# fverdoja/Fast-3D-Pointcloud-Segmentation

Measured on AMD Instinct MI355X. Metric: Mpoints/sec segmented end-to-end, 1M-pt RGB-D frames, higher is better.
Workload: dtype f32

## Files before the change

fast-3d-pointcloud-segmentation_amd/csrc/f3ds_kernels.inc:

```


namespace {

struct P16 { float x, y, z; uint32_t rgba; };

struct DevCounters {
    unsigned long long n_finite;
    uint32_t bbox[6];
    uint32_t bbox_any;
    uint32_t n_valid;
    uint32_t n_voxels;
    uint32_t n_cells;
    uint32_t n_seeds;
    uint32_t n_edges;
    uint32_t n_alive;
    uint32_t n_merges;
    uint32_t n_regions;
    uint32_t n_events;
    int error;
    int r_overflow;
    float lambda;
    uint32_t seg_count;
    uint32_t n_ghosts;
    int depth;
// ... 94 lines not shown
            uint32_t v[16];
            if (i0 + 15u < m) {
#pragma unroll
                for (int q = 0; q < 4; ++q) { const uint4 x = *reinterpret_cast<const uint4*>(data + i0 + 4 * q); v[4 * q] = x.x; v[4 * q + 1] = x.y; v[4 * q + 2] = x.z; v[4 * q + 3] = x.w; }
            } else {
#pragma unroll
                for (int k = 0; k < 16; ++k) v[k] = i0 + k < m ? data[i0 + k] : 0u;
            }
            uint32_t sum = 0;
#pragma unroll
            for (int k = 0; k < 16; ++k) sum += v[k];
            uint32_t tot;
            const uint32_t inc = block_incl_scan<256>(sum, &tot);
            uint32_t run = carry + inc - sum;
            if (i0 + 15u < m) {
#pragma unroll
                for (int q = 0; q < 4; ++q) {
                    uint4 x; x.x = run; x.y = run + v[4 * q]; x.z = x.y + v[4 * q + 1]; x.w = x.z + v[4 * q + 2]; run = x.w + v[4 * q + 3];
                    *reinterpret_cast<uint4*>(data + i0 + 4 * q) = x;
                }
            } else {
#pragma unroll
                for (int k = 0; k < 16; ++k) if (i0 + k < m) { data[i0 + k] = run; run += v[k]; }
            }
            carry += tot;
        }
    }
};
struct d_scan_tiles {
    static constexpr int BLOCK = SCAN_THREADS;
    __device__ void operator()(const uint32_t* in, uint32_t* out, uint32_t* tile_sums, uint32_t n) const {
        if (BIX > 0 && BIX * SCAN_TILE >= n) return;
        const uint32_t base = BIX * SCAN_TILE + threadIdx.x * SCAN_ITEMS;
        uint32_t v[SCAN_ITEMS];
        uint32_t s = 0;
    #pragma unroll
        for (int i = 0; i < SCAN_ITEMS; ++i) { v[i] = (base + i < n) ? in[base + i] : 0u; s += v[i]; }
        uint32_t tot;
        uint32_t inc = block_incl_scan<SCAN_THREADS>(s, &tot);
        uint32_t run = inc - s;
    #pragma unroll
        for (int i = 0; i < SCAN_ITEMS; ++i) { run += v[i]; if (base + i < n) out[base + i] = run; }
        if (threadIdx.x == 0) tile_sums[BIX] = tot;
    }
};
struct d_scan_add {
    static constexpr int BLOCK = SCAN_THREADS;
    __device__ void operator()(uint32_t* out, const uint32_t* tile_offsets, uint32_t n) const {
        if (BIX > 0 && BIX * SCAN_TILE >= n) return;
        const uint32_t base = BIX * SCAN_TILE + threadIdx.x * SCAN_ITEMS;
        const uint32_t off = tile_offsets[BIX];
    #pragma unroll
        for (int i = 0; i < SCAN_ITEMS; ++i) if (base + i < n) out[base + i] += off;
    }
};

constexpr int RS_THREADS = 256;
constexpr int RS_WAVES = RS_THREADS / 64;
constexpr int RS_STRIPS = 16;
constexpr int RS_TILE = RS_THREADS * RS_STRIPS;
constexpr int RS_MAXBITS = 9;
constexpr int RS_BINS = 1 << RS_MAXBITS;

struct d_radix_hist {
    static constexpr int BLOCK = RS_THREADS;
    __device__ void operator()(const uint64_t* keys, uint32_t n, int shift, int bits, uint32_t* hist,
                                                         uint32_t nblocks, const uint32_t* n_dev) const {
        if (BIX >= nblocks) return;
        if (n_dev) { const uint32_t nd = *n_dev; n = nd < n ? nd : n; }
        __shared__ uint32_t lh[RS_BINS];
        for (int i = threadIdx.x; i < RS_BINS; i += RS_THREADS) lh[i] = 0;
        __syncthreads();
        const uint32_t mask = (1u << bits) - 1u;
        const uint32_t wbase = BIX * RS_TILE + (threadIdx.x >> 6) * (64 * RS_STRIPS);
    #pragma unroll
        for (int s = 0; s < RS_STRIPS; ++s) {
            uint32_t i = wbase + s * 64 + lane_id();
            if (i < n) atomicAdd(&lh[(uint32_t)(keys[i] >> shift) & mask], 1u);
        }
        __syncthreads();
        for (uint32_t d = threadIdx.x; d < (1u << bits); d += RS_THREADS) hist[d * nblocks + BIX] = lh[d];
    }
};
struct d_radix_scatter {
    static constexpr int BLOCK = RS_THREADS;
    __device__ void operator()(const uint64_t* keys, const uint32_t* vals, uint64_t* keys_out,
                                                            uint32_t* vals_out, uint32_t n, int shift, int bits,
                                                            const uint32_t* hist_scanned, uint32_t nblocks, const uint32_t* n_dev) const {
        if (BIX >= nblocks) return;
        if (n_dev) { const uint32_t nd = *n_dev; n = nd < n ? nd : n; }
        __shared__ uint32_t wcount[RS_WAVES][RS_BINS];
        const uint32_t mask = (1u << bits) - 1u;
        const int w = threadIdx.x >> 6;
        for (int i = threadIdx.x; i < RS_WAVES * RS_BINS; i += RS_THREADS) (&wcount[0][0])[i] = 0;
        __syncthreads();
        const uint32_t wbase = BIX * RS_TILE + w * (64 * RS_STRIPS);
        uint64_t k[RS_STRIPS];
    #pragma unroll
        for (int s = 0; s < RS_STRIPS; ++s) {
            uint32_t i = wbase + s * 64 + lane_id();
            k[s] = i < n ? keys[i] : 0ull;
            if (i < n) atomicAdd(&wcount[w][(uint32_t)(k[s] >> shift) & mask], 1u);
        }
        __syncthreads();
        for (uint32_t d = threadIdx.x; d < (1u << bits); d += RS_THREADS) {
            uint32_t run = hist_scanned[d * nblocks + BIX];
            for (int ww = 0; ww < RS_WAVES; ++ww) { uint32_t t = wcount[ww][d]; wcount[ww][d] = run; run += t; }
        }
        __syncthreads();
    #pragma unroll
        for (int s = 0; s < RS_STRIPS; ++s) {
            uint32_t i = wbase + s * 64 + lane_id();
            const bool valid = i < n;
            const uint32_t d = (uint32_t)(k[s] >> shift) & mask;
            uint64_t peers = __ballot(valid);
            for (int b = 0; b < bits; ++b) {
                uint64_t m = __ballot(valid && ((d >> b) & 1u));
                peers &= ((d >> b) & 1u) ? m : ~m;
            }
            uint32_t pos = 0;
            if (valid) pos = wcount[w][d] + (uint32_t)__popcll(peers & lanemask_lt());
            __builtin_amdgcn_wave_barrier();
            if (valid && (peers & lanemask_lt()) == 0ull) wcount[w][d] += (uint32_t)__popcll(peers);
            __builtin_amdgcn_wave_barrier();
            if (valid) { keys_out[pos] = k[s]; vals_out[pos] = vals[i]; }
        }
    }
};


struct d_radix_scatter_k {
    static constexpr int BLOCK = RS_THREADS;
    __device__ void operator()(const uint64_t* keys, uint64_t* keys_out, uint32_t n, int shift, int bits, const uint32_t* hist_scanned, uint32_t nblocks) const {
        if (BIX >= nblocks) return;
        __shared__ uint32_t wcount[RS_WAVES][RS_BINS];
        const uint32_t mask = (1u << bits) - 1u;
        const int w = threadIdx.x >> 6;
        for (int i = threadIdx.x; i < RS_WAVES * RS_BINS; i += RS_THREADS) (&wcount[0][0])[i] = 0;
        __syncthreads();
        const uint32_t wbase = BIX * RS_TILE + w * (64 * RS_STRIPS);
        uint64_t k[RS_STRIPS];
    #pragma unroll
        for (int s = 0; s < RS_STRIPS; ++s) {
            uint32_t i = wbase + s * 64 + lane_id();
            k[s] = i < n ? keys[i] : 0ull;
            if (i < n) atomicAdd(&wcount[w][(uint32_t)(k[s] >> shift) & mask], 1u);
        }
        __syncthreads();
        for (uint32_t d = threadIdx.x; d < (1u << bits); d += RS_THREADS) {
            uint32_t run = hist_scanned[d * nblocks + BIX];
            for (int ww = 0; ww < RS_WAVES; ++ww) { uint32_t t = wcount[ww][d]; wcount[ww][d] = run; run += t; }
        }
        __syncthreads();
    #pragma unroll
        for (int s = 0; s < RS_STRIPS; ++s) {
            uint32_t i = wbase + s * 64 + lane_id();
            const bool valid = i < n;
            const uint32_t d = (uint32_t)(k[s] >> shift) & mask;
            uint64_t peers = __ballot(valid);
            for (int b = 0; b < bits; ++b) {
                uint64_t m = __ballot(valid && ((d >> b) & 1u));
                peers &= ((d >> b) & 1u) ? m : ~m;
            }
            uint32_t pos = 0;
            if (valid) pos = wcount[w][d] + (uint32_t)__popcll(peers & lanemask_lt());
            __builtin_amdgcn_wave_barrier();
            if (valid && (peers & lanemask_lt()) == 0ull) wcount[w][d] += (uint32_t)__popcll(peers);
            __builtin_amdgcn_wave_barrier();
            if (valid) keys_out[pos] = k[s];
        }
    }
};

struct FrameArgs {
    int use_transform, fold_negative_z, leaf_order;
    float voxel_res, seed_res, w_color, w_spatial, w_normal;
};

__device__ inline P16 load_point(const P16* pts, size_t i) {
    const uint4 q = reinterpret_cast<const uint4*>(pts)[i];
    P16 p;
    p.x = __uint_as_float(q.x); p.y = __uint_as_float(q.y); p.z = __uint_as_float(q.z); p.rgba = q.w;
    return p;
}

__device__ inline bool vt_blocks(int depth) { return depth <= N_BLOCK_DEPTH_MAX; }
constexpr uint32_t BT_EMPTY = 0xFFFFFFFFu;
struct __attribute__((aligned(16))) BtEntry { uint32_t key, base; unsigned long long vacant; };
static_assert(sizeof(BtEntry) == 16, "one 16-byte load per probe");
template <class T> __device__ inline bool vt_cas(T* p, T* expect, T v, bool agent) {
    return agent ? __hip_atomic_compare_exchange_strong(p, expect, v, __ATOMIC_RELAXED, __ATOMIC_RELAXED, __HIP_MEMORY_SCOPE_AGENT)
                 : __hip_atomic_compare_exchange_strong(p, expect, v, __ATOMIC_RELAXED, __ATOMIC_RELAXED, __HIP_MEMORY_SCOPE_WORKGROUP);
}
__device__ inline void vt_insert(uint64_t* hkeys, uint32_t* hvals, uint32_t hmask, bool agent, unsigned x, unsigned y, unsigned z, uint32_t v) {
    const unsigned long long pk = (unsigned long long)n_pack_key(x, y, z);
    uint32_t h = (uint32_t)hash64((uint64_t)pk) & hmask;
    for (;;) {
        unsigned long long expect = HASH_EMPTY;
        if (vt_cas((unsigned long long*)&hkeys[h], &expect, pk, agent) || expect == pk) { hvals[h] = v; return; }
        h = (h + 1u) & hmask;
    }
}
__device__ inline int vt_find(const uint64_t* hkeys, const uint32_t* hvals, uint32_t hmask, unsigned x, unsigned y, unsigned z) {
    const uint64_t pk = n_pack_key(x, y, z);
    uint32_t h = (uint32_t)hash64(pk) & hmask;
    for (;;) {
        const uint64_t k = hkeys[h];
        if (k == pk) return (int)hvals[h];
        if (k == HASH_EMPTY) return -1;
        h = (h + 1u) & hmask;
    }
}
__device__ inline BtEntry* bt_entry(BtEntry* tab, uint32_t tmask, bool agent, uint32_t bk) {
    uint32_t h = (uint32_t)hash64((uint64_t)bk) & tmask;
    for (;;) {
        uint32_t expect = BT_EMPTY;
        if (vt_cas(&tab[h].key, &expect, bk, agent) || expect == bk) return &tab[h];
        h = (h + 1u) & tmask;
    }
}
__device__ inline int bt_find(const BtEntry* tab, uint32_t tmask, int leaf_order, unsigned x, unsigned y, unsigned z) {
    const uint32_t bk = n_block_key(x, y, z);
    uint32_t h = (uint32_t)hash64((uint64_t)bk) & tmask;
    for (;;) {
        const uint4 e = reinterpret_cast<const uint4*>(tab)[h];
        if (e.x == bk) return n_block_ordinal(e.y, ~(((uint64_t)e.w << 32) | (uint64_t)e.z), n_block_cell(x, y, z), leaf_order);
        if (e.x == BT_EMPTY) return -1;
        h = (h + 1u) & tmask;
    }
}
struct RgbdArgs {
    uint32_t width, n;
    uint32_t depth_pitch, color_pitch;
    int depth_f32, color_format;
    float depth_scale, fx, fy, cx, cy;
};
template <class T> __device__ inline T load_unaligned(const unsigned char* p) { T t; __builtin_memcpy(&t, p, sizeof(T)); return t; }
template <bool DEPTH_F32, int COLOR>
__device__ inline void deproject_loop(const unsigned char* depth, const unsigned char* color, const RgbdArgs& a, P16* out) {
    const uint32_t stride = gridDim.x * blockDim.x;
    const uint32_t sv = stride / a.width, su = stride - sv * a.width;
    uint32_t i = BIX * blockDim.x + threadIdx.x;
    uint32_t v = i / a.width, u = i - v * a.width;
    for (; i < a.n; i += stride) {
        const unsigned char* drow = depth + (size_t)v * a.depth_pitch;
        const unsigned char* crow = color + (size_t)v * a.color_pitch;
        float z = 0.0f;
        bool valid;
        if constexpr (DEPTH_F32) valid = n_depth_to_z(reinterpret_cast<const float*>(drow)[u], a.depth_scale, z);
        else valid = n_depth_to_z(reinterpret_cast<const uint16_t*>(drow)[u], a.depth_scale, z);
        uint32_t rgba;
        if constexpr (COLOR == 0) { const unsigned char* p = crow + 3u * (size_t)u; rgba = n_color_word(p[0], p[1], p[2], 255u); }
        else {
            const uint32_t w = load_unaligned<uint32_t>(crow + 4u * (size_t)u);
            rgba = COLOR == 1 ? n_color_word(w & 255u, (w >> 8) & 255u, (w >> 16) & 255u, w >> 24) : w;
        }
        float x, y, zo;
        n_deproject(u, v, valid, z, a.fx, a.fy, a.cx, a.cy, x, y, zo);
        reinterpret_cast<uint4*>(out)[i] = make_uint4(__float_as_uint(x), __float_as_uint(y), __float_as_uint(zo), rgba);
        u += su; v += sv;
        if (u >= a.width) { u -= a.width; ++v; }
    }
}
struct d_deproject {
    static constexpr int BLOCK = 256;
    __device__ void operator()(const unsigned char* depth, const unsigned char* color, RgbdArgs a, P16* out) const {
        if (a.depth_f32) {
            if (a.color_format == 0) deproject_loop<true, 0>(depth, color, a, out);
            else if (a.color_format == 1) deproject_loop<true, 1>(depth, color, a, out);
            else deproject_loop<true, 2>(depth, color, a, out);
        } else {
            if (a.color_format == 0) deproject_loop<false, 0>(depth, color, a, out);
            else if (a.color_format == 1) deproject_loop<false, 1>(depth, color, a, out);
            else deproject_loop<false, 2>(depth, color, a, out);
        }
    }
};
struct d_bbox {
    static constexpr int BLOCK = 256;
    __device__ void operator()(const P16* pts, uint32_t n, FrameArgs fa, DevCounters* dc) const {
        float mn[3] = {F3DS_FLT_MAX, F3DS_FLT_MAX, F3DS_FLT_MAX}, mx[3] = {-F3DS_FLT_MAX, -F3DS_FLT_MAX, -F3DS_FLT_MAX};
        uint32_t nfin = 0, any = 0;
        for (uint32_t i = BIX * blockDim.x + threadIdx.x; i < n; i += gridDim.x * blockDim.x) {
            P16 p = load_point(pts, i);
            float x = p.x, y = p.y, z = p.z;
            n_prelude(z, fa.fold_negative_z);
            if (n_finite3(x, y, z)) nfin++;
            n_transform(x, y, z, fa.use_transform);
            if (!n_finite3(x, y, z)) continue;
            any = 1;
            if (x < mn[0]) mn[0] = x;
            if (y < mn[1]) mn[1] = y;
            if (z < mn[2]) mn[2] = z;
            if (x > mx[0]) mx[0] = x;
            if (y > mx[1]) mx[1] = y;
            if (z > mx[2]) mx[2] = z;
        }
    #pragma unroll
        for (int d = 32; d >= 1; d >>= 1) {
            for (int a = 0; a < 3; ++a) {
                float t = __shfl_xor(mn[a], d, 64); if (t < mn[a]) mn[a] = t;
                t = __shfl_xor(mx[a], d, 64); if (t > mx[a]) mx[a] = t;
            }
            nfin += __shfl_xor(nfin, d, 64);
            any |= __shfl_xor(any, d, 64);
        }
        __shared__ float smn[4][3], smx[4][3];
        __shared__ uint32_t sfin[4], sany[4];
        const int w = threadIdx.x >> 6;
        if (lane_id() == 0) { for (int a = 0; a < 3; ++a) { smn[w][a] = mn[a]; smx[w][a] = mx[a]; } sfin[w] = nfin; sany[w] = any; }
// ... 513 lines not shown
                    const unsigned long long o = __shfl_down(m, d, 64);
                    if (lane + d < 64u && !(ahead & ((1ull << d) - 1ull))) m |= o;
                }
                if (in && (head || lane == 0u)) {
                    BtEntry* const e = bt_entry(tab, hmask, agent, bk);
                    if (agent) __hip_atomic_fetch_and(&e->vacant, ~m, __ATOMIC_RELAXED, __HIP_MEMORY_SCOPE_AGENT);
                    else __hip_atomic_fetch_and(&e->vacant, ~m, __ATOMIC_RELAXED, __HIP_MEMORY_SCOPE_WORKGROUP);
                    if (head) e->base = v;
                }
            }
        }
    }
};
struct d_voxel_list_accum {
    static constexpr int BLOCK = 256;
    __device__ void operator()(const P16* pts, uint32_t* list, const uint32_t* seg_start, FrameArgs fa, float* vf, uint32_t* vcount, DevCounters* dc, uint32_t capV) const {
        __shared__ __attribute__((aligned(16))) uint4 buf[VG_CHUNK];
        if (dc->ev_overflow) return;
        const uint32_t V = dc->n_voxels < capV ? dc->n_voxels : capV;
        const bool disorder = dc->vox_disorder != 0u;
        const uint32_t tid = threadIdx.x;
        for (uint32_t vb = BIX * 256u; vb < V; vb += gridDim.x * 256u) {
            const uint32_t v = vb + tid;
            const bool mine = v < V;
            const uint32_t s = mine ? seg_start[v] : 0u, e = mine ? seg_start[v + 1] : 0u;
            const uint32_t p0 = seg_start[vb], p1 = seg_start[vb + 256u < V ? vb + 256u : V];
            if (__syncthreads_or(e - s > VL_MAX_RUN)) { if (tid == 0) { dc->error = F3DS_ERR_UNSUPPORTED; dc->ev_overflow = 6; } return; }
            if (disorder) {
                for (uint32_t a = s + 1u; a < e; ++a) {
                    const uint32_t x = list[a];
                    uint32_t b = a;
                    while (b > s && list[b - 1u] > x) { list[b] = list[b - 1u]; --b; }
                    if (b != a) list[b] = x;
                }
                __threadfence_block();
                __syncthreads();
            }
            float sx = 0, sy = 0, sz = 0, sr = 0, sg = 0, sb = 0;
            for (uint32_t c0 = p0; c0 < p1; c0 += VG_CHUNK) {
                const uint32_t c1 = p1 - c0 < VG_CHUNK ? p1 : c0 + VG_CHUNK;
                uint32_t idx[VG_CHUNK / 256];
        #pragma unroll
                for (uint32_t j = 0; j < VG_CHUNK / 256; ++j) { const uint32_t i = c0 + j * 256u + tid; idx[j] = list[i < c1 ? i : c1 - 1u]; }
                uint4 q[VG_CHUNK / 256];
        #pragma unroll
                for (uint32_t j = 0; j < VG_CHUNK / 256; ++j) q[j] = reinterpret_cast<const uint4*>(pts)[idx[j]];
        #pragma unroll
                for (uint32_t j = 0; j < VG_CHUNK / 256; ++j) buf[j * 256u + tid] = q[j];
                __syncthreads();
                const uint32_t a = s > c0 ? s : c0, b = e < c1 ? e : c1;
                for (uint32_t i = a; i < b; ++i) {
                    const uint4 w = buf[i - c0];
                    float z = __uint_as_float(w.z); n_prelude(z, fa.fold_negative_z);
                    sx += __uint_as_float(w.x); sy += __uint_as_float(w.y); sz += z;
                    sr += (float)((w.w >> 16) & 255u); sg += (float)((w.w >> 8) & 255u); sb += (float)(w.w & 255u);
                }
                __syncthreads();
            }
            if (!mine) continue;
            const float c = (float)(e - s);
            vcount[v] = e - s;
            float4* row = reinterpret_cast<float4*>(vf + (size_t)v * 12);
            row[0] = make_float4(sx / c, sy / c, sz / c, sr / c);
            row[1] = make_float4(sg / c, sb / c, 0.0f, 0.0f);
            row[2] = make_float4(0.0f, 0.0f, 0.0f, 0.0f);
        }
    }
};
__device__ inline int hash_find(const uint64_t* hkeys, const uint32_t* hvals, uint32_t hmask, uint64_t pk) {
    uint32_t h = (uint32_t)hash64(pk) & hmask;
    for (;;) {
        uint64_t k = hkeys[h];
        if (k == pk) return (int)hvals[h];
        if (k == HASH_EMPTY) return -1;
        h = (h + 1u) & hmask;
    }
}

struct d_neighbors {
    static constexpr int BLOCK = 256;
    __device__ void operator()(const uint32_t* vkey, const DevCounters* dc, const GridInfo* gp, int leaf_order, const uint64_t* hkeys,
                                                  const uint32_t* hvals, uint32_t hmask, int* nbr, int* nbrT) const {
        __shared__ int tr[27][65];
        const uint32_t V = dc->n_voxels;
        const unsigned max_key = gp->max_key;
        const bool blocks = vt_blocks(gp->depth);
        const BtEntry* const tab = reinterpret_cast<const BtEntry*>(hkeys);
        for (uint32_t vb = BIX * 64u; vb < V; vb += gridDim.x * 64u) {
            const uint32_t nv = V - vb < 64u ? V - vb : 64u, np = nv * 27u;
            for (uint32_t tl = threadIdx.x; tl < np; tl += 256u) {
                const uint32_t vl = tl / 27u, s = tl - vl * 27u, v = vb + vl;
                const int d[3] = {(int)(s / 9u) - 1, (int)((s / 3u) % 3u) - 1, (int)(s % 3u) - 1};
                bool ok = true; unsigned k[3];
                for (int a = 0; a < 3; ++a) {
                    long long q = (long long)vkey[v * 3 + a] + d[a];
                    if (q < 0 || q > (long long)max_key) ok = false;
                    k[a] = (unsigned)q;
                }
                const int u = !ok ? -1 : blocks ? bt_find(tab, hmask, leaf_order, k[0], k[1], k[2]) : vt_find(hkeys, hvals, hmask, k[0], k[1], k[2]);
                nbr[(size_t)vb * 27u + tl] = u;
                tr[s][vl] = u;
            }
            __syncthreads();
            for (uint32_t r = threadIdx.x; r < 27u * 64u; r += 256u) {
                const uint32_t s = r >> 6, vl = r & 63u;
                if (vl < nv) nbrT[(size_t)s * V + vb + vl] = tr[s][vl];
            }
            __syncthreads();
        }
    }
};
constexpr int NT_TILE = 128;
constexpr int NT_HCAP = 2048;
#ifndef F3DS_NT_SLOTS
#define F3DS_NT_SLOTS 896
#endif
#ifndef F3DS_NT_RING1
#define F3DS_NT_RING1 448
#endif
constexpr int NT_SLOTS = F3DS_NT_SLOTS;
constexpr int NT_RING1 = F3DS_NT_RING1;
constexpr uint16_t NT_NONE = 0xFFFFu;
constexpr uint32_t NT_HNONE = 0x3FFu;
constexpr uint32_t NT_ORD_LIMIT = (1u << 22) - 2u;
static_assert(NT_SLOTS < 1023, "slot numbers share a word with the ordinal");
constexpr uint16_t NT_ZERO = NT_SLOTS;
constexpr uint32_t SW_TILE_NONE = 0xFFFFFFFFu;
constexpr int SW_SLOT_BITS = 9;
constexpr int SW_SLOT_WORDS = (27 * SW_SLOT_BITS + 31) / 32;
static_assert(NT_RING1 < (1 << SW_SLOT_BITS), "a list position must fit its bit field");
__device__ __forceinline__ void sw_slots_pack(const uint32_t pos[27], uint32_t w[SW_SLOT_WORDS]) {
#pragma unroll
    for (int k = 0; k < SW_SLOT_WORDS; ++k) w[k] = 0u;
#pragma unroll
    for (int j = 0; j < 27; ++j) {
        const int bit = j * SW_SLOT_BITS, wi = bit >> 5, sh = bit & 31;
        w[wi] |= pos[j] << sh;
        if (sh + SW_SLOT_BITS > 32) w[wi + 1] |= pos[j] >> (32 - sh);
    }
}
__device__ __forceinline__ uint32_t sw_slot(const uint32_t w[SW_SLOT_WORDS], int j) {
    const int bit = j * SW_SLOT_BITS, wi = bit >> 5, sh = bit & 31;
    uint32_t x = w[wi] >> sh;
    if (sh + SW_SLOT_BITS > 32) x |= w[wi + 1] << (32 - sh);
    return x & ((1u << SW_SLOT_BITS) - 1u);
}
__device__ inline void cov_add(float acc[9], const float4 q) {
    acc[0] += q.x * q.x; acc[1] += q.x * q.y; acc[2] += q.x * q.z;
    acc[3] += q.y * q.y; acc[4] += q.y * q.z; acc[5] += q.z * q.z;
    acc[6] += q.x; acc[7] += q.y; acc[8] += q.z;
}
__device__ __forceinline__ uint32_t lds_addr(const float* p);
typedef float f3ds_f2 __attribute__((ext_vector_type(2)));
typedef float f3ds_f4 __attribute__((ext_vector_type(4)));
struct CovPairs {
    f3ds_f2 a0, a1, a2, a3; float sz;
    __device__ void zero() { a0 = a1 = a2 = a3 = f3ds_f2{0.0f, 0.0f}; sz = 0.0f; }
    __device__ void add(const f3ds_f4 q) {
        const f3ds_f2 xy = q.xy, zy = q.zw;
        a0 += xy * q.xx;
        a1 += xy * q.zz;
        a2 += zy * zy;
        a3 += xy;
        sz += q.z;
    }
    __device__ void store(float acc[9]) const { acc[0] = a0.x; acc[1] = a0.y; acc[2] = a1.x; acc[3] = a2.y; acc[4] = a1.y; acc[5] = a2.x; acc[6] = a3.x; acc[7] = a3.y; acc[8] = sz; }
};
template <int NTT>
struct d_normals_t {
    static constexpr int BLOCK = NTT;
    static constexpr int PT = (NT_RING1 * 27 + NTT - 1) / NTT;
    static constexpr int PR = PT % 9 == 0 ? 9 : (PT % 8 == 0 ? 8 : (PT % 6 == 0 ? 6 : (PT % 4 == 0 ? 4 : (PT % 3 == 0 ? 3 : (PT % 2 == 0 ? 2 : 1)))));
#ifndef F3DS_NORMALS_WPS
#define F3DS_NORMALS_WPS 3
#endif
#ifndef F3DS_NORMALS_WPS256
#define F3DS_NORMALS_WPS256 3
#endif
    static constexpr int WAVES_PER_SIMD = NTT > 256 ? F3DS_NORMALS_WPS : F3DS_NORMALS_WPS256;
    __device__ static uint32_t hslot(uint32_t ord) { return (ord * 2654435761u) >> 21; }
    __device__ void one_tile(const uint32_t bix, float* vf, const int* nbr, const DevCounters* dc, uint32_t* tile_n1, uint32_t* tile_ord, uint32_t* tile_slots, uint32_t holes) const {
        __shared__ uint32_t hw[NT_HCAP];
// ... 2987 lines not shown
```

fast-3d-pointcloud-segmentation_amd/csrc/f3ds_numerics.h:

```cpp
#ifndef F3DS_NUMERICS_H_
#define F3DS_NUMERICS_H_

#include "f3ds_math.h"

namespace f3ds {

#define F3DS_FLT_MAX 3.402823466e+38f
#define F3DS_FLT_MIN 1.175494351e-38f
#define F3DS_FLT_EPS 1.192092896e-07f

F3DS_HD float n_sqrtf(float x) { return __builtin_sqrtf(x); }
F3DS_HD double n_sqrt(double x) { return __builtin_sqrt(x); }
F3DS_HD bool n_finite3(float x, float y, float z) { return m_isfinitef(x) && m_isfinitef(y) && m_isfinitef(z); }
F3DS_HD float n_nanf() { return m_from_bitsf(0x7fc00000u); }

struct GridInfo {
    double min[3];
    double max[3];
    double res;
    int depth;
    unsigned max_key;
    int error;
    int empty;
};
// ... 31 lines not shown
        if (k > mk) mk = k;
    }
    double lg = m_log((double)mk) / m_log(2.0) - eps;
    unsigned d = (unsigned)__builtin_ceil(lg);
    if (d > 32u) d = 32u;
    if (d > 21u) { g.error = -4; g.depth = (int)d; return; }
    g.depth = (int)d;
    g.max_key = (1u << d) - 1u;
    double side = (double)(1u << d) * g.res;
    for (int a = 0; a < 3; ++a) {
        double over = (side - (g.max[a] - g.min[a])) / 2.0;
        if (over > eps) { g.min[a] -= over; g.max[a] += over; }
    }
}
F3DS_HD void n_grid_from_bbox(const float mn[3], const float mx[3], float voxel_res, GridInfo& g) {
    g.error = 0; g.empty = 0; g.depth = 0; g.max_key = 0;
    g.res = (double)voxel_res;
    for (int a = 0; a < 3; ++a) {
        double lo = (double)mn[a], hi = (double)mx[a];
        g.min[a] = lo < hi ? lo : hi;
        g.max[a] = lo < hi ? hi : lo;
    }
    n_key_bit_size(g);
}
F3DS_HD void n_point_key(const GridInfo& g, float x, float y, float z, int use_transform, unsigned key[3]) {
    n_transform(x, y, z, use_transform);
    if (!use_transform || n_finite3(x, y, z)) {
        const double inv = 1.0 / g.res;
        const float p[3] = {x, y, z};
        for (int a = 0; a < 3; ++a) {
            const double d = (double)p[a] - g.min[a];
            const double q1 = d * inv;
            const unsigned k1 = (unsigned)q1;
            const double f = q1 - (double)k1;
            key[a] = (f > 1e-6 && f < 1.0 - 1e-6 && q1 < 4194304.0) ? k1 : (unsigned)(d / g.res);
        }
    } else {
        key[0] = key[1] = key[2] = 0u;
    }
}
F3DS_HD uint32_t n_spread3_10(uint32_t v) {
    v = (v | (v << 16)) & 0x030000FFu;
    v = (v | (v << 8)) & 0x0300F00Fu;
    v = (v | (v << 4)) & 0x030C30C3u;
    v = (v | (v << 2)) & 0x09249249u;
    return v;
}
F3DS_HD uint64_t n_spread3_21(uint64_t v) {
    v = (v | (v << 32)) & 0x001F00000000FFFFull;
    v = (v | (v << 16)) & 0x001F0000FF0000FFull;
    v = (v | (v << 8)) & 0x100F00F00F00F00Full;
    v = (v | (v << 4)) & 0x10C30C30C30C30C3ull;
    v = (v | (v << 2)) & 0x1249249249249249ull;
    return v;
}
F3DS_HD uint64_t n_morton(unsigned x, unsigned y, unsigned z, int depth) {
    if (depth <= 10) {
        const uint32_t m = (1u << depth) - 1u;
        return (uint64_t)((n_spread3_10(x & m) << 2) | (n_spread3_10(y & m) << 1) | n_spread3_10(z & m));
    }
    const uint64_t m = (1ull << depth) - 1ull;
    return (n_spread3_21(x & m) << 2) | (n_spread3_21(y & m) << 1) | n_spread3_21(z & m);
}
F3DS_HD void n_demorton(uint64_t c, int depth, unsigned key[3]) {
    unsigned x = 0, y = 0, z = 0;
    for (int b = depth - 1; b >= 0; --b) {
        unsigned d = (unsigned)(c >> (3 * b)) & 7u;
        x = (x << 1) | ((d >> 2) & 1u);
        y = (y << 1) | ((d >> 1) & 1u);
        z = (z << 1) | (d & 1u);
    }
    key[0] = x; key[1] = y; key[2] = z;
}
F3DS_HD uint64_t n_pack_key(unsigned x, unsigned y, unsigned z) {
    return ((uint64_t)x << 42) | ((uint64_t)y << 21) | (uint64_t)z;
}
#define N_BLOCK_DEPTH_MAX 12
F3DS_HD uint32_t n_block_key(unsigned x, unsigned y, unsigned z) { return ((x >> 2) << 20) | ((y >> 2) << 10) | (z >> 2); }
F3DS_HD unsigned n_block_cell(unsigned x, unsigned y, unsigned z) { return (unsigned)n_morton(x & 3u, y & 3u, z & 3u, 2); }
F3DS_HD int n_block_ordinal(uint32_t base, uint64_t mask, unsigned cell, int leaf_order) {
    if (!((mask >> cell) & 1ull)) return -1;
    const uint64_t before = leaf_order == 1 ? ((mask >> cell) >> 1) : (mask & ((1ull << cell) - 1ull));
    return (int)(base + (uint32_t)__builtin_popcountll(before));
}

F3DS_HD void n_roots2(float b, float c, float r[3]) {
    r[0] = 0.0f;
    float d = (float)((double)(b * b) - 4.0 * (double)c);
    if (d < 0.0f) d = 0.0f;
    float sd = n_sqrtf(d);
    r[2] = 0.5f * (b + sd);
    r[1] = 0.5f * (b - sd);
}
template <class K = m_lit> F3DS_HD void n_roots(float m00, float m01, float m02, float m11, float m12, float m22, float r[3], K mc = K()) {
    float c0 = m00 * m11 * m22 + 2.0f * m01 * m02 * m12 - m00 * m12 * m12 - m11 * m02 * m02 - m22 * m01 * m01;
    float c1 = m00 * m11 - m01 * m01 + m00 * m22 - m02 * m02 + m11 * m22 - m12 * m12;
    float c2 = m00 + m11 + m22;
    if (m_absf(c0) < F3DS_FLT_EPS) { n_roots2(c2, c1, r); return; }
    const float inv3 = (float)(1.0 / 3.0);
    const float sqrt3 = 1.7320508075688772f;
    float c2_3 = c2 * inv3;
    float a_3 = (c1 - c2 * c2_3) * inv3;
    if (a_3 > 0.0f) a_3 = 0.0f;
    float half_b = 0.5f * (c0 + c2_3 * (2.0f * c2_3 * c2_3 - c1));
    float q = half_b * half_b + a_3 * a_3 * a_3;
    if (q > 0.0f) q = 0.0f;
    float rho = n_sqrtf(-a_3);
    float theta = m_atan2f(n_sqrtf(-q), half_b, mc) * inv3;
    float ct = m_cosf(theta, mc), st = m_sinf(theta, mc);
    r[0] = c2_3 + 2.0f * rho * ct;
    r[1] = c2_3 - rho * (ct + sqrt3 * st);
    r[2] = c2_3 - rho * (ct - sqrt3 * st);
    float t;
    if (r[0] >= r[1]) { t = r[0]; r[0] = r[1]; r[1] = t; }
    if (r[1] >= r[2]) {
        t = r[1]; r[1] = r[2]; r[2] = t;
        if (r[0] >= r[1]) { t = r[0]; r[0] = r[1]; r[1] = t; }
    }
    if (r[0] <= 0.0f) n_roots2(c2, c1, r);
}
F3DS_HD float n_sum3(float a, float b, float c) { return a + (b + c); }
F3DS_HD void n_cross(float a0, float a1, float a2, float b0, float b1, float b2, float o[3]) {
    o[0] = a1 * b2 - a2 * b1;
    o[1] = a2 * b0 - a0 * b2;
    o[2] = a0 * b1 - a1 * b0;
}
F3DS_HD void n_plane_normal(const float accu_raw[9], unsigned count, const float view_point[3], float out[4]) {
    float nx, ny, nz, nw;
    if (count < 3u) {
        nx = ny = nz = nw = n_nanf();
    } else {
        float cnt = (float)count;
        float a[9];
        for (int i = 0; i < 9; ++i) a[i] = accu_raw[i] / cnt;
        float c00 = a[0] - a[6] * a[6], c01 = a[1] - a[6] * a[7], c02 = a[2] - a[6] * a[8];
        float c11 = a[3] - a[7] * a[7], c12 = a[4] - a[7] * a[8], c22 = a[5] - a[8] * a[8];
        float scale = m_absf(c00);
        float t;
        t = m_absf(c01); if (t > scale) scale = t;
        t = m_absf(c02); if (t > scale) scale = t;
        t = m_absf(c11); if (t > scale) scale = t;
        t = m_absf(c12); if (t > scale) scale = t;
        t = m_absf(c22); if (t > scale) scale = t;
        if (scale <= F3DS_FLT_MIN) scale = 1.0f;
        float m00 = c00 / scale, m01 = c01 / scale, m02 = c02 / scale, m11 = c11 / scale, m12 = c12 / scale, m22 = c22 / scale;
        float r[3];
        n_roots(m00, m01, m02, m11, m12, m22, r);
        m00 -= r[0]; m11 -= r[0]; m22 -= r[0];
        float v1[3], v2[3], v3[3];
        n_cross(m00, m01, m02, m01, m11, m12, v1);
        n_cross(m00, m01, m02, m02, m12, m22, v2);
        n_cross(m01, m11, m12, m02, m12, m22, v3);
        float l1 = n_sum3(v1[0] * v1[0], v1[1] * v1[1], v1[2] * v1[2]);
        float l2 = n_sum3(v2[0] * v2[0], v2[1] * v2[1], v2[2] * v2[2]);
        float l3 = n_sum3(v3[0] * v3[0], v3[1] * v3[1], v3[2] * v3[2]);
        const float* v; float l;
        if (l1 >= l2 && l1 >= l3) { v = v1; l = l1; }
        else if (l2 >= l1 && l2 >= l3) { v = v2; l = l2; }
        else { v = v3; l = l3; }
        float s = n_sqrtf(l);
        nx = v[0] / s; ny = v[1] / s; nz = v[2] / s;
        nw = -1.0f * ((nx * a[6] + ny * a[7]) + (nz * a[8] + 0.0f * 1.0f));
    }
    float cos_theta = ((0.0f - view_point[0]) * nx + (0.0f - view_point[1]) * ny) + ((0.0f - view_point[2]) * nz + 0.0f * nw);
    if (cos_theta < 0.0f) { nx *= -1.0f; ny *= -1.0f; nz *= -1.0f; }
    float z = (nx * nx + ny * ny) + (nz * nz + 0.0f);
// ... 138 lines not shown
```

Baseline: 3738.

## Stage radix scatter through LDS and dedupe block-table lookups per voxel

Radix scatter now ranks keys locally, stages them in shared memory in bucket order, and writes them out contiguously using per-digit global offsets, so global stores are coalesced instead of scattered. The neighbour-table kernel now resolves at most 8 block-hash entries per voxel (one per octant) into shared memory and derives all 27 neighbours from them, instead of probing the hash table 27 times. In exchange there is more shared memory, extra barriers, and a block scan in the scatter.

```diff
diff --git a/fast-3d-pointcloud-segmentation_amd/csrc/f3ds_kernels.inc b/fast-3d-pointcloud-segmentation_amd/csrc/f3ds_kernels.inc
--- a/fast-3d-pointcloud-segmentation_amd/csrc/f3ds_kernels.inc
+++ b/fast-3d-pointcloud-segmentation_amd/csrc/f3ds_kernels.inc
@@ -200,6 +200,86 @@
         for (uint32_t d = threadIdx.x; d < (1u << bits); d += RS_THREADS) hist[d * nblocks + BIX] = lh[d];
     }
 };
+#ifndef F3DS_RS_STAGE
+#define F3DS_RS_STAGE 1024
+#endif
+constexpr int RS_STAGE = F3DS_RS_STAGE;
+static_assert(RS_STAGE >= RS_THREADS && RS_TILE % RS_STAGE == 0, "the whole tile or an even part of it");
+template <bool PAIRS>
+__device__ inline void radix_scatter_tile(const uint64_t* keys, const uint32_t* vals, uint64_t* keys_out, uint32_t* vals_out, uint32_t n, int shift, int bits,
+                                          const uint32_t* hist_scanned, uint32_t nblocks) {
+    __shared__ uint32_t wcount[RS_WAVES][RS_BINS];
+    __shared__ uint32_t gofs[RS_BINS];
+    __shared__ uint64_t skey[RS_STAGE];
+    __shared__ uint32_t sval[PAIRS ? RS_STAGE : 1];
+    const uint32_t tbase = BIX * RS_TILE;
+    if (tbase >= n) return;
+    const uint32_t nt = n - tbase < (uint32_t)RS_TILE ? n - tbase : (uint32_t)RS_TILE;
+    const uint32_t mask = (1u << bits) - 1u;
+    const int w = threadIdx.x >> 6;
+    for (int i = threadIdx.x; i < RS_WAVES * RS_BINS; i += RS_THREADS) (&wcount[0][0])[i] = 0;
+    __syncthreads();
+    const uint32_t wbase = tbase + w * (64 * RS_STRIPS);
+    uint64_t k[RS_STRIPS];
+    uint32_t v[PAIRS ? RS_STRIPS : 1];
+#pragma unroll
+    for (int s = 0; s < RS_STRIPS; ++s) {
+        uint32_t i = wbase + s * 64 + lane_id();
+        k[s] = i < n ? keys[i] : 0ull;
+        if (PAIRS) v[s] = i < n ? vals[i] : 0u;
+        if (i < n) atomicAdd(&wcount[w][(uint32_t)(k[s] >> shift) & mask], 1u);
+    }
+    __syncthreads();
+    {
+        const uint32_t d0 = threadIdx.x * 2u;
+        uint32_t c[2] = {0u, 0u};
+        for (int j = 0; j < 2; ++j) for (int ww = 0; ww < RS_WAVES; ++ww) c[j] += wcount[ww][d0 + j];
+        uint32_t tot;
+        uint32_t run = block_incl_scan<RS_THREADS>(c[0] + c[1], &tot) - (c[0] + c[1]);
+        for (int j = 0; j < 2; ++j) {
+            const uint32_t d = d0 + j;
+            if (d <= mask) gofs[d] = hist_scanned[d * nblocks + BIX] - run;
+            for (int ww = 0; ww < RS_WAVES; ++ww) { uint32_t t = wcount[ww][d]; wcount[ww][d] = run; run += t; }
+        }
+    }
+    __syncthreads();
+    uint32_t pos[RS_STRIPS];
+#pragma unroll
+    for (int s = 0; s < RS_STRIPS; ++s) {
+        uint32_t i = wbase + s * 64 + lane_id();
+        const bool valid = i < n;
+        const uint32_t d = (uint32_t)(k[s] >> shift) & mask;
+        uint64_t peers = __ballot(valid);
+        for (int b = 0; b < bits; ++b) {
+            uint64_t m = __ballot(valid && ((d >> b) & 1u));
+            peers &= ((d >> b) & 1u) ? m : ~m;
+        }
+        uint32_t p = 0xFFFFFFFFu;
+        if (valid) p = wcount[w][d] + (uint32_t)__popcll(peers & lanemask_lt());
+        __builtin_amdgcn_wave_barrier();
+        if (valid && (peers & lanemask_lt()) == 0ull) wcount[w][d] += (uint32_t)__popcll(peers);
+        __builtin_amdgcn_wave_barrier();
+        pos[s] = p;
+        if (p < (uint32_t)RS_STAGE) { skey[p] = k[s]; if (PAIRS) sval[p] = v[s]; }
+    }
+#pragma unroll
+    for (uint32_t r0 = 0; r0 < (uint32_t)RS_TILE; r0 += RS_STAGE) {
+        if (r0 >= nt) break;
+        if (r0) {
+            __syncthreads();
+#pragma unroll
+            for (int s = 0; s < RS_STRIPS; ++s) if (pos[s] - r0 < (uint32_t)RS_STAGE) { skey[pos[s] - r0] = k[s]; if (PAIRS) sval[pos[s] - r0] = v[s]; }
+        }
+        __syncthreads();
+        const uint32_t m = nt - r0 < (uint32_t)RS_STAGE ? nt - r0 : (uint32_t)RS_STAGE;
+        for (uint32_t j = threadIdx.x; j < m; j += RS_THREADS) {
+            const uint64_t key = skey[j];
+            const uint32_t o = gofs[(uint32_t)(key >> shift) & mask] + r0 + j;
+            keys_out[o] = key;
+            if (PAIRS) vals_out[o] = sval[j];
+        }
+    }
+}
 struct d_radix_scatter {
     static constexpr int BLOCK = RS_THREADS;
     __device__ void operator()(const uint64_t* keys, const uint32_t* vals, uint64_t* keys_out,
@@ -207,86 +287,14 @@
                                                             const uint32_t* hist_scanned, uint32_t nblocks, const uint32_t* n_dev) const {
         if (BIX >= nblocks) return;
         if (n_dev) { const uint32_t nd = *n_dev; n = nd < n ? nd : n; }
-        __shared__ uint32_t wcount[RS_WAVES][RS_BINS];
-        const uint32_t mask = (1u << bits) - 1u;
-        const int w = threadIdx.x >> 6;
-        for (int i = threadIdx.x; i < RS_WAVES * RS_BINS; i += RS_THREADS) (&wcount[0][0])[i] = 0;
-        __syncthreads();
-        const uint32_t wbase = BIX * RS_TILE + w * (64 * RS_STRIPS);
-        uint64_t k[RS_STRIPS];
-    #pragma unroll
-        for (int s = 0; s < RS_STRIPS; ++s) {
-            uint32_t i = wbase + s * 64 + lane_id();
-            k[s] = i < n ? keys[i] : 0ull;
-            if (i < n) atomicAdd(&wcount[w][(uint32_t)(k[s] >> shift) & mask], 1u);
-        }
-        __syncthreads();
-        for (uint32_t d = threadIdx.x; d < (1u << bits); d += RS_THREADS) {
-            uint32_t run = hist_scanned[d * nblocks + BIX];
-            for (int ww = 0; ww < RS_WAVES; ++ww) { uint32_t t = wcount[ww][d]; wcount[ww][d] = run; run += t; }
-        }
-        __syncthreads();
-    #pragma unroll
-        for (int s = 0; s < RS_STRIPS; ++s) {
-            uint32_t i = wbase + s * 64 + lane_id();
-            const bool valid = i < n;
-            const uint32_t d = (uint32_t)(k[s] >> shift) & mask;
-            uint64_t peers = __ballot(valid);
-            for (int b = 0; b < bits; ++b) {
-                uint64_t m = __ballot(valid && ((d >> b) & 1u));
-                peers &= ((d >> b) & 1u) ? m : ~m;
-            }
-            uint32_t pos = 0;
-            if (valid) pos = wcount[w][d] + (uint32_t)__popcll(peers & lanemask_lt());
-            __builtin_amdgcn_wave_barrier();
-            if (valid && (peers & lanemask_lt()) == 0ull) wcount[w][d] += (uint32_t)__popcll(peers);
-            __builtin_amdgcn_wave_barrier();
-            if (valid) { keys_out[pos] = k[s]; vals_out[pos] = vals[i]; }
-        }
-    }
-};
-
-
+        radix_scatter_tile<true>(keys, vals, keys_out, vals_out, n, shift, bits, hist_scanned, nblocks);
+    }
+};
 struct d_radix_scatter_k {
     static constexpr int BLOCK = RS_THREADS;
     __device__ void operator()(const uint64_t* keys, uint64_t* keys_out, uint32_t n, int shift, int bits, const uint32_t* hist_scanned, uint32_t nblocks) const {
         if (BIX >= nblocks) return;
-        __shared__ uint32_t wcount[RS_WAVES][RS_BINS];
-        const uint32_t mask = (1u << bits) - 1u;
-        const int w = threadIdx.x >> 6;
-        for (int i = threadIdx.x; i < RS_WAVES * RS_BINS; i += RS_THREADS) (&wcount[0][0])[i] = 0;
-        __syncthreads();
-        const uint32_t wbase = BIX * RS_TILE + w * (64 * RS_STRIPS);
-        uint64_t k[RS_STRIPS];
-    #pragma unroll
-        for (int s = 0; s < RS_STRIPS; ++s) {
-            uint32_t i = wbase + s * 64 + lane_id();
-            k[s] = i < n ? keys[i] : 0ull;
-            if (i < n) atomicAdd(&wcount[w][(uint32_t)(k[s] >> shift) & mask], 1u);
-        }
-        __syncthreads();
-        for (uint32_t d = threadIdx.x; d < (1u << bits); d += RS_THREADS) {
-            uint32_t run = hist_scanned[d * nblocks + BIX];
-            for (int ww = 0; ww < RS_WAVES; ++ww) { uint32_t t = wcount[ww][d]; wcount[ww][d] = run; run += t; }
-        }
-        __syncthreads();
-    #pragma unroll
-        for (int s = 0; s < RS_STRIPS; ++s) {
-            uint32_t i = wbase + s * 64 + lane_id();
-            const bool valid = i < n;
-            const uint32_t d = (uint32_t)(k[s] >> shift) & mask;
-            uint64_t peers = __ballot(valid);
-            for (int b = 0; b < bits; ++b) {
-                uint64_t m = __ballot(valid && ((d >> b) & 1u));
-                peers &= ((d >> b) & 1u) ? m : ~m;
-            }
-            uint32_t pos = 0;
-            if (valid) pos = wcount[w][d] + (uint32_t)__popcll(peers & lanemask_lt());
-            __builtin_amdgcn_wave_barrier();
-            if (valid && (peers & lanemask_lt()) == 0ull) wcount[w][d] += (uint32_t)__popcll(peers);
-            __builtin_amdgcn_wave_barrier();
-            if (valid) keys_out[pos] = k[s];
-        }
+        radix_scatter_tile<false>(keys, nullptr, keys_out, nullptr, n, shift, bits, hist_scanned, nblocks);
     }
 };
 
@@ -337,13 +345,12 @@
         h = (h + 1u) & tmask;
     }
 }
-__device__ inline int bt_find(const BtEntry* tab, uint32_t tmask, int leaf_order, unsigned x, unsigned y, unsigned z) {
-    const uint32_t bk = n_block_key(x, y, z);
+__device__ inline uint4 bt_find(const BtEntry* tab, uint32_t tmask, uint32_t bk) {
     uint32_t h = (uint32_t)hash64((uint64_t)bk) & tmask;
     for (;;) {
         const uint4 e = reinterpret_cast<const uint4*>(tab)[h];
-        if (e.x == bk) return n_block_ordinal(e.y, ~(((uint64_t)e.w << 32) | (uint64_t)e.z), n_block_cell(x, y, z), leaf_order);
-        if (e.x == BT_EMPTY) return -1;
+        if (e.x == bk) return e;
+        if (e.x == BT_EMPTY) return make_uint4(BT_EMPTY, 0u, 0xFFFFFFFFu, 0xFFFFFFFFu);
         h = (h + 1u) & tmask;
     }
 }
@@ -1023,22 +1030,50 @@
     __device__ void operator()(const uint32_t* vkey, const DevCounters* dc, const GridInfo* gp, int leaf_order, const uint64_t* hkeys,
                                                   const uint32_t* hvals, uint32_t hmask, int* nbr, int* nbrT) const {
         __shared__ int tr[27][65];
+        __shared__ uint4 ent[64][8];
+        __shared__ unsigned vk[64][3];
         const uint32_t V = dc->n_voxels;
         const unsigned max_key = gp->max_key;
         const bool blocks = vt_blocks(gp->depth);
         const BtEntry* const tab = reinterpret_cast<const BtEntry*>(hkeys);
         for (uint32_t vb = BIX * 64u; vb < V; vb += gridDim.x * 64u) {
             const uint32_t nv = V - vb < 64u ? V - vb : 64u, np = nv * 27u;
+            if (blocks) {
+                const uint32_t vl = threadIdx.x >> 2, q = threadIdx.x & 3u;
+                if (vl < nv) {
+                    unsigned key[3];
+                    for (int a = 0; a < 3; ++a) key[a] = vkey[(vb + vl) * 3 + a];
+                    if (q < 3u) vk[vl][q] = key[q];
+                    for (unsigned xb = 0; xb < 2u; ++xb) {
+                        const unsigned o = (xb << 2) | q;
+                        unsigned slot, cell; uint32_t bk;
+                        uint4 e = make_uint4(BT_EMPTY, 0u, 0xFFFFFFFFu, 0xFFFFFFFFu);
+                        if (n_octant_slot(key, o, slot) && n_neighbor_cell(key, max_key, slot, bk, cell)) e = bt_find(tab, hmask, bk);
+                        ent[vl][o] = e;
+                    }
+                }
+                __syncthreads();
+            }
             for (uint32_t tl = threadIdx.x; tl < np; tl += 256u) {
                 const uint32_t vl = tl / 27u, s = tl - vl * 27u, v = vb + vl;
-                const int d[3] = {(int)(s / 9u) - 1, (int)((s / 3u) % 3u) - 1, (int)(s % 3u) - 1};
-                bool ok = true; unsigned k[3];
-                for (int a = 0; a < 3; ++a) {
-                    long long q = (long long)vkey[v * 3 + a] + d[a];
-                    if (q < 0 || q > (long long)max_key) ok = false;
-                    k[a] = (unsigned)q;
-                }
-                const int u = !ok ? -1 : blocks ? bt_find(tab, hmask, leaf_order, k[0], k[1], k[2]) : vt_find(hkeys, hvals, hmask, k[0], k[1], k[2]);
+                int u = -1;
+                if (blocks) {
+                    const unsigned key[3] = {vk[vl][0], vk[vl][1], vk[vl][2]};
+                    unsigned cell; uint32_t bk;
+                    if (n_neighbor_cell(key, max_key, s, bk, cell)) {
+                        const uint4 e = ent[vl][n_neighbor_octant(key, s)];
+                        u = n_block_ordinal(e.y, ~(((uint64_t)e.w << 32) | (uint64_t)e.z), cell, leaf_order);
+                    }
+                } else {
+                    const int d[3] = {(int)(s / 9u) - 1, (int)((s / 3u) % 3u) - 1, (int)(s % 3u) - 1};
+                    bool ok = true; unsigned k[3];
+                    for (int a = 0; a < 3; ++a) {
+                        long long q = (long long)vkey[v * 3 + a] + d[a];
+                        if (q < 0 || q > (long long)max_key) ok = false;
+                        k[a] = (unsigned)q;
+                    }
+                    if (ok) u = vt_find(hkeys, hvals, hmask, k[0], k[1], k[2]);
+                }
                 nbr[(size_t)vb * 27u + tl] = u;
                 tr[s][vl] = u;
             }
diff --git a/fast-3d-pointcloud-segmentation_amd/csrc/f3ds_numerics.h b/fast-3d-pointcloud-segmentation_amd/csrc/f3ds_numerics.h
--- a/fast-3d-pointcloud-segmentation_amd/csrc/f3ds_numerics.h
+++ b/fast-3d-pointcloud-segmentation_amd/csrc/f3ds_numerics.h
@@ -137,6 +137,37 @@
     if (!((mask >> cell) & 1ull)) return -1;
     const uint64_t before = leaf_order == 1 ? ((mask >> cell) >> 1) : (mask & ((1ull << cell) - 1ull));
     return (int)(base + (uint32_t)__builtin_popcountll(before));
+}
+F3DS_HD bool n_neighbor_cell(const unsigned key[3], unsigned max_key, unsigned slot, uint32_t& bk, unsigned& cell) {
+    const int d[3] = {(int)(slot / 9u) - 1, (int)((slot / 3u) % 3u) - 1, (int)(slot % 3u) - 1};
+    bool ok = true; unsigned k[3];
+    for (int a = 0; a < 3; ++a) {
+        const long long q = (long long)key[a] + d[a];
+        if (q < 0 || q > (long long)max_key) ok = false;
+        k[a] = (unsigned)q;
+    }
+    bk = n_block_key(k[0], k[1], k[2]); cell = n_block_cell(k[0], k[1], k[2]);
+    return ok;
+}
+F3DS_HD unsigned n_neighbor_octant(const unsigned key[3], unsigned slot) {
+    const int d[3] = {(int)(slot / 9u) - 1, (int)((slot / 3u) % 3u) - 1, (int)(slot % 3u) - 1};
+    unsigned o = 0;
+    for (int a = 0; a < 3; ++a) {
+        const int t = (int)(key[a] & 3u) + d[a];
+        o = (o << 1) | (t < 0 || t > 3 ? 1u : 0u);
+    }
+    return o;
+}
+F3DS_HD bool n_octant_slot(const unsigned key[3], unsigned octant, unsigned& slot) {
+    bool any = true; unsigned s = 0;
+    for (int a = 0; a < 3; ++a) {
+        const unsigned lo = key[a] & 3u;
+        int d = 0;
+        if ((octant >> (2 - a)) & 1u) { d = lo == 0u ? -1 : 1; if (lo != 0u && lo != 3u) any = false; }
+        s = s * 3u + (unsigned)(d + 1);
+    }
+    slot = s;
+    return any;
 }
 
 F3DS_HD void n_roots2(float b, float c, float r[3]) {
```

Measured after the change: 3726. No clear change (-0.3%).
